# RicoFio/disentangle_mlp

Measured on AMD Instinct MI355X. Metric: celeba64_betavaegan_train_images_per_sec, higher is better.
Workload: dtype fp32-equivalent (fp16x3 split of fp32 operands on the f16 MFMA, fp32 accumulate, every convolution and the Linear layers with >= 2^20 weights (vg_gemm_nt_f16x3); the small Linear layers (vendor GEMMs), BatchNorm, losses, Adam in fp32)

## Files before the change

disentangle_mlp_amd/csrc/common.hpp:

```cpp
#pragma once
#include <hip/hip_runtime.h>
#include <stdint.h>

typedef float f32x16 __attribute__((ext_vector_type(16)));
typedef float f32x4 __attribute__((ext_vector_type(4)));

#define VG_WAVE 64

#ifdef VG_TUNING
#define VG_KNOB(type, name, value) type name = value
#else
#define VG_KNOB(type, name, value) constexpr type name = value
#endif

#define VG_CHECK_LAUNCH()                         \
  do {                                            \
    hipError_t e__ = hipGetLastError();           \
    if (e__ != hipSuccess) return (int)e__;       \
  } while (0)

__device__ __forceinline__ f32x16 mfma32(float a, float b, f32x16 c) {
  return __builtin_amdgcn_mfma_f32_32x32x2f32(a, b, c, 0, 0, 0);
}

__device__ __forceinline__ int acc_row(int r, int lane) {
  return (r & 3) + 8 * (r >> 2) + 4 * (lane >> 5);
}

__device__ __forceinline__ float act_slope(float v, float slope) { return v * (v > 0.f ? 1.f : slope); }

typedef __attribute__((ext_vector_type(8))) __bf16 bf16x8;
typedef __attribute__((ext_vector_type(8))) _Float16 f16x8;

#define VG_PLANES_F16_FLAG 0x100

constexpr int VG_PACK_SPARE = 6;
constexpr size_t vg_pack_trailer_units(int nsteps, int planes, int CoutP) {
  return (size_t)(nsteps + VG_PACK_SPARE) * planes * 2 * CoutP;
}

constexpr int VG_STATS_SLOT_DEPTH = 16;

__device__ __forceinline__ unsigned f16_bound_exp(float amax) {
  const unsigned e = (__float_as_uint(amax) >> 23) & 0xffu;
  return min(max(e, 15u), 254u);
}
__device__ __forceinline__ float f16_scale_of(float amax) { return __uint_as_float((268u - f16_bound_exp(amax)) << 23); }
__device__ __forceinline__ float f16_unscale_of(float amax) { return __uint_as_float((f16_bound_exp(amax) - 14u) << 23); }

template <int NP, bool F16>
__device__ __forceinline__ void split_planes16(float* v, f32x4* out) {
  if constexpr (F16) {
    static_assert(NP == 2, "fp16 planes: hi + lo");
    typedef float f32x2 __attribute__((ext_vector_type(2)));
    typedef _Float16 f16x2 __attribute__((ext_vector_type(2)));
    f16x2 hi[4], lo[4];
#pragma unroll
    for (int j = 0; j < 4; ++j) {
      const f32x2 v2 = {v[2 * j], v[2 * j + 1]};
      const f16x2 h = __builtin_convertvector(v2, f16x2);
      hi[j] = h;
      lo[j] = __builtin_convertvector(v2 - __builtin_convertvector(h, f32x2), f16x2);
    }
    struct P4 { f16x2 q[4]; };
    out[0] = __builtin_bit_cast(f32x4, P4{{hi[0], hi[1], hi[2], hi[3]}});
    out[1] = __builtin_bit_cast(f32x4, P4{{lo[0], lo[1], lo[2], lo[3]}});
  } else {
#pragma unroll
    for (int p = 0; p < NP; ++p) {
      bf16x8 q;
#pragma unroll
      for (int j = 0; j < 8; ++j) {
        const __bf16 h = (__bf16)v[j];
        q[j] = h;
        v[j] -= (float)h;
      }
      out[p] = __builtin_bit_cast(f32x4, q);
    }
  }
}

template <bool F16>
__device__ __forceinline__ f32x16 mfma_split16(bf16x8 a, bf16x8 b, f32x16 c) {
  if constexpr (F16)
    return __builtin_amdgcn_mfma_f32_32x32x16_f16(__builtin_bit_cast(f16x8, a), __builtin_bit_cast(f16x8, b), c, 0, 0, 0);
  else
    return __builtin_amdgcn_mfma_f32_32x32x16_bf16(a, b, c, 0, 0, 0);
}

template <typename T>
__device__ __forceinline__ T wave_sum(T v) {
#pragma unroll
  for (int o = 32; o > 0; o >>= 1) v += __shfl_down(v, o, 64);
  return v;
}

template <typename T>
__device__ __forceinline__ T wave_allsum(T v) {
#pragma unroll
  for (int o = 32; o > 0; o >>= 1) v += __shfl_xor(v, o, 64);
  return v;
}

template <int NT, typename T>
__device__ __forceinline__ T block_sum(T v, T* red) {
  v = wave_sum(v);
  const int lane = threadIdx.x & 63, wid = threadIdx.x >> 6;
  __syncthreads();
  if (lane == 0) red[wid] = v;
  __syncthreads();
  T t = 0;
  if (threadIdx.x == 0) {
#pragma unroll
    for (int i = 0; i < NT / 64; ++i) t += red[i];
  }
  return t;
}

__device__ __forceinline__ unsigned abs_bits(float v) { return __float_as_uint(v) & 0x7fffffffu; }

template <int NT>
__device__ __forceinline__ void block_amax_atomic(unsigned m, unsigned* out) {
  __shared__ unsigned amax_red[NT / 64];
#pragma unroll
  for (int o = 32; o > 0; o >>= 1) m = max(m, (unsigned)__shfl_xor((int)m, o, 64));
  const int lane = threadIdx.x & 63, wid = threadIdx.x >> 6;
  if (lane == 0) amax_red[wid] = m;
  __syncthreads();
  if (threadIdx.x == 0) {
#pragma unroll
    for (int i = 1; i < NT / 64; ++i) m = max(m, amax_red[i]);
    if (m > __hip_atomic_load(out, __ATOMIC_RELAXED, __HIP_MEMORY_SCOPE_AGENT)) atomicMax(out, m);
  }
}

__host__ __device__ constexpr int cdiv(int a, int b) { return (a + b - 1) / b; }

int vg_internal_wgrad_reduce(const float* slabs, float* dw, int n, int splits, hipStream_t st, int accumulate = 0);
size_t vg_internal_ring_workspace_bytes(int mode, int B, int Cin, int H, int W, int Cout, int planes);
size_t vg_internal_ring_stats_floats(int mode, int B, int Cin, int H, int W, int Cout, int planes);
int vg_internal_ring_conv(int mode, const float* x, const void* packed, const float* bias, float* y, int B, int Cin, int H,
                          int W, int Cout, int planes, void* workspace, size_t workspace_bytes, const float* in_scale,
                          const float* in_shift, int in_act, float* stats, size_t stats_floats, const float* in_amax,
                          hipStream_t st);
#ifdef VG_TUNING
void vg_internal_ring_set_variant(int v);
void vg_internal_wx_set_th(int th);
#endif
int vg_internal_convT_s1_thin(const float* x, const float* w, const float* bias, float* y, int B, int Cin, int H,
                              int W, int Cout, hipStream_t st);
```

disentangle_mlp_amd/csrc/conv_ring.hip:

```cpp
#include "common.hpp"
#include "vaegan_hip.h"

namespace {

enum { R_FWD = 0, R_TR = 1 };
constexpr int RNT = 512;
#ifndef VG_RING_SLOTS
#define VG_RING_SLOTS 3
#endif
#ifndef VG_RING_NOPF
#define VG_RING_NOPF 0
#endif
constexpr int ring_slots(bool f16, int slotu, int patchu) {
  if (!f16) return 3;
  int n = VG_RING_SLOTS;
  while (n > 3 && (n * slotu + patchu + 1) * 16 > 160 * 1024) --n;
  return n;
}
static_assert(VG_RING_SLOTS >= 3 && VG_RING_SLOTS <= VG_PACK_SPARE, "ring depth");

constexpr int ring_cols(int mode, int TW, int PW) {
  if (mode == R_FWD) {
    const int need = (PW + 1) / 2;
    if (TW == 8) { int c = need; while ((c & 3) != 2) ++c; return c; }
    return (need + 3) & ~3;
  }
  if (TW == 16) return (PW + 15) & ~15;
  if (TW == 8) { int c = PW; while ((c & 15) != 8) ++c; return c; }
  return (PW + 3) & ~3;
}

template <int MODE_, int NB_, int TH_, int TW_, int WC_, int FC_, int FP_, int NP_, bool F16_ = false>
struct RCfg {
  static constexpr int MODE = MODE_, NB = NB_, TH = TH_, TW = TW_, WC = WC_, WP = 8 / WC_, FC = FC_, FP = FP_, NP = NP_;
  static constexpr bool F16 = F16_;
  static_assert(!F16_ || NP_ == 2, "fp16 planes: hi + lo");
  static constexpr int S = 2;
  static constexpr int TN = 32 * WC * FC, TM = NB * TH * TW;
  static constexpr int NTMAX = (MODE == R_FWD) ? 5 : 3;
  static constexpr int PH = (MODE == R_FWD) ? S * (TH - 1) + 5 : TH + NTMAX - 1;
  static constexpr int PW = (MODE == R_FWD) ? S * (TW - 1) + 5 : TW + NTMAX - 1;
  static constexpr int COLS = ring_cols(MODE, TW, PW);
  static constexpr int ROWU = (MODE == R_FWD) ? 2 * COLS : COLS;
  static constexpr int IMGU = NB * PH * ROWU;
  static constexpr int BUFU = (MODE == R_FWD) ? NP * IMGU : NP * 2 * IMGU;
  static constexpr int PATCHU = 2 * BUFU;
  static constexpr int SLOTU = NP * 2 * TN;
  static constexpr int NSLOT = ring_slots(F16_, SLOTU, PATCHU);
  static constexpr int RINGU = NSLOT * SLOTU;
  static constexpr int LDSU = RINGU + PATCHU + 1;
  static constexpr int DMA_TOTAL = SLOTU / 64;
  static constexpr int NDMA = (DMA_TOTAL + 7) / 8;
  static constexpr int NPIX = NB * PH * PW;
  static constexpr int NQ = ((MODE == R_FWD) ? 1 : 2) * ((NPIX + RNT - 1) / RNT);
  static constexpr int NL = NQ * 8;
  static constexpr int NCLS = (MODE == R_FWD) ? 1 : 4;
  static_assert(TM == 32 * WP * FP, "pixel tile");
  static_assert(FP + 5 <= VG_STATS_SLOT_DEPTH, "statistics slot: an fma chain of FP, 5 butterfly additions");
  static_assert(WC == 1 || WC == 2 || WC == 4 || WC == 8, "wavefront grid");
  static_assert(SLOTU % 64 == 0, "a step's filter slice is whole DMA instructions");
  static_assert(LDSU * 16 <= 160 * 1024, "LDS");
};

struct RArgs {
  const float* x;
  const bf16x8* w;
  const float* bias;
  float* y;
  int B, Cin, XH, XW, Cout, CoutP, YH, YW;
  int ntiles_n, tiles_w, tiles_hw, blocks_per_cls;
  int cps;
  size_t ysplit;
  const float* in_scale;
  const float* in_shift;
  int in_act;
  float* stats;
  const float* in_amax;
  const float* w_unscale;
  int paired;
};

__host__ __device__ constexpr int tr_taps_before(int R, int SS) {
  int n = 0;
  for (int r = 0; r < 2; ++r)
    for (int s = 0; s < 2; ++s) {
      if (r == R && s == SS) return n;
      n += ((5 - r + 1) / 2) * ((5 - s + 1) / 2);
    }
  return n;
}

template <int N>
__device__ __forceinline__ void wait_vmcnt() {
  static_assert(N >= 0 && N < 64, "vmcnt is a 6-bit counter");
  asm volatile("s_waitcnt vmcnt(%0)" ::"n"(N) : "memory");
}

template <class C, int R, int SS, bool AFF, int R2 = -1, int SS2 = -1>
__device__ __forceinline__ void ring_body(const RArgs& A, f32x4* lds, int bid, int split) {
  constexpr int MODE = C::MODE, S = C::S, NB = C::NB, TH = C::TH, TW = C::TW, PH = C::PH, PW = C::PW;
  constexpr int COLS = C::COLS, ROWU = C::ROWU, IMGU = C::IMGU, NQ = C::NQ, FC = C::FC, FP = C::FP, NP = C::NP;
  constexpr int NTMAX = C::NTMAX, BUFU = C::BUFU, SLOTU = C::SLOTU, NDMA = C::NDMA, NL = C::NL, TN = C::TN;
  constexpr int NSLOT = C::NSLOT;
  constexpr bool F16 = C::F16;
  constexpr int NTH = (MODE == R_FWD) ? 5 : (5 - R + 1) / 2;
  constexpr int NTW = (MODE == R_FWD) ? 5 : (5 - SS + 1) / 2;
  constexpr bool TWO = R2 >= 0;
  static_assert(!TWO || MODE == R_TR, "two classes: transposed form");
  constexpr int NTH2 = TWO ? (5 - R2 + 1) / 2 : 0, NTW2 = TWO ? (5 - SS2 + 1) / 2 : 1;
  constexpr int NA = NTH * NTW, NB2 = NTH2 * NTW2;
  constexpr int NSTEP = NA + NB2;
  constexpr int NACC = TWO ? 2 : 1;
  static_assert(!TWO || NA >= NSLOT, "the prologue's DMAs all belong to the first class");
  constexpr int PSTEP = (MODE == R_FWD) ? S : 1;
  constexpr int RING0 = 0, PATCH0 = C::RINGU, DUMMY = C::RINGU + C::PATCHU;

  const int tid = threadIdx.x, lane = tid & 63;
  const int wid = __builtin_amdgcn_readfirstlane(tid >> 6);
  const int kb = lane >> 5, l32 = lane & 31;
  const int wc = wid % C::WC, wp = wid / C::WC;
  int nt, pt;
  {
    const int ntn = A.ntiles_n, npatch = A.blocks_per_cls / ntn, full = (npatch / 8) * 8 * ntn;
    if (bid < full) {
      const int xcd = bid & 7, j = bid >> 3;
      pt = xcd * (npatch / 8) + j / ntn;
      nt = j % ntn;
    } else {
      const int t = bid - full;
      pt = (npatch / 8) * 8 + t / ntn;
      nt = t % ntn;
    }
  }
  const int sp = pt % A.tiles_hw, bg = pt / A.tiles_hw;
  const int th0 = (sp / A.tiles_w) * TH, tw0 = (sp % A.tiles_w) * TW;
  const int b0 = bg * NB, n0 = nt * TN;
  const int Cin = A.Cin, Cout = A.Cout, XH = A.XH, XW = A.XW, HW = XH * XW;
  const int ih0 = (MODE == R_FWD) ? th0 * S - 2 : th0 - (NTMAX - 1 - 2 / S);
  const int iw0 = (MODE == R_FWD) ? tw0 * S - 2 : tw0 - (NTMAX - 1 - 2 / S);
  const float* xb = A.x + (size_t)b0 * Cin * HW;

  struct Unit {
    unsigned ofs;
    int dst;
    bool ok;
  };
  auto unit_of = [&](int q) -> Unit {
    int t0 = tid;
    asm volatile("" : "+v"(t0));
    const int kbs = (MODE == R_FWD) ? 0 : (q & 1);
    const int e = t0 + ((MODE == R_FWD) ? q : (q >> 1)) * RNT;
    const int col = e % PW;
    int t = e / PW;
    const int r = t % PH;
    t /= PH;
    const int nb = t % NB;
    const int ih = ih0 + r, iw = iw0 + col;
    const bool in = e < C::NPIX;
    Unit u;
    u.ok = in && ih >= 0 && ih < XH && iw >= 0 && iw < XW && (b0 + nb) < A.B;
    const int nbc = min(nb, A.B - 1 - b0), ihc = min(max(ih, 0), XH - 1), iwc = min(max(iw, 0), XW - 1);
    u.ofs = 4u * (unsigned)((nbc * Cin + kbs * 8) * HW + ihc * XW + iwc);
    u.dst = in ? kbs * IMGU + (nb * PH + r) * ROWU + ((MODE == R_FWD) ? (col & 1) * COLS + (col >> 1) : col) : -1;
    return u;
  };

  float preg[NQ][8];
  int staged_c0 = 0;
  const float aff_slope = A.in_act == VG_ACT_NONE ? 1.f : (A.in_act == VG_ACT_RELU ? 0.f : 0.2f);
  float x_scale = 1.f, x_unscale = 1.f;
  if constexpr (F16) {
    const float amax = *A.in_amax;
    x_scale = f16_scale_of(amax);
    x_unscale = f16_unscale_of(amax);
  }
  auto stage_load = [&](int c0) {
    c0 = min(c0, Cin - ((MODE == R_FWD) ? 8 : 16));
    staged_c0 = c0;
    unsigned ofs[NQ];
#pragma unroll
    for (int q = 0; q < NQ; ++q) ofs[q] = unit_of(q).ofs;
#pragma unroll
    for (int j = 0; j < 8; ++j) {
      const char* xj = (const char*)(xb + (size_t)(c0 + j) * HW);
#pragma unroll
      for (int q = 0; q < NQ; ++q) preg[q][j] = *(const float*)(xj + ofs[q]);
    }
  };
  auto split_unit = [&](int q, int bufu) {
    const Unit u = unit_of(q);
    f32x4 pl[NP];
    float vv[8];
    const int cb = __builtin_amdgcn_readfirstlane(staged_c0 + ((MODE == R_FWD) ? 0 : (q & 1) * 8));
#pragma unroll
    for (int j = 0; j < 8; ++j) {
      float v = preg[q][j];
      if constexpr (AFF) {
        v = fmaf(v, A.in_scale[cb + j], A.in_shift[cb + j]);
        v = act_slope(v, aff_slope);
      }
      v = u.ok ? v : 0.f;
      vv[j] = F16 ? v * x_scale : v;
    }
    split_planes16<NP, F16>(vv, pl);
    const int d = PATCH0 + bufu + u.dst;
#pragma unroll
    for (int p = 0; p < NP; ++p)
      lds[(u.dst >= 0) ? d + p * ((MODE == R_FWD) ? IMGU : 2 * IMGU) : DUMMY] = pl[p];
  };
  auto stage_store = [&](int bufu) {
#pragma unroll
    for (int q = 0; q < NQ; ++q) split_unit(q, bufu);
  };

  const int CoutP = A.CoutP;
  const size_t wstep = (size_t)2 * NP * CoutP;
  const int nchunks = Cin / 16;
  const bf16x8* wcls = A.w + (size_t)((MODE == R_FWD) ? 0 : tr_taps_before(R, SS)) * nchunks * wstep;
  const bf16x8* dma_ptr2 = A.w + (size_t)(TWO ? tr_taps_before(R2 < 0 ? 0 : R2, SS2 < 0 ? 0 : SS2) : 0) * nchunks * wstep;
  unsigned dma_src[NDMA];
  int dma_dst[NDMA];
#pragma unroll
  for (int j = 0; j < NDMA; ++j) {
    const int i = (wid * NDMA + j) % C::DMA_TOTAL;
    const int u = i * 64 + lane;
    const int row = u / TN, col = u % TN;
    dma_src[j] = 16u * (unsigned)(row * CoutP + n0 + col);
    dma_dst[j] = i * 64;
  }
  const bf16x8* dma_ptr1 = wcls;
  auto dma_next = [&](int slot, bool second = false) {
    const bf16x8*& dma_ptr = second ? dma_ptr2 : dma_ptr1;
#pragma unroll
    for (int j = 0; j < NDMA; ++j) {
      const unsigned m0v = (unsigned)(size_t)(__attribute__((address_space(3))) void*)(lds + RING0 + slot * SLOTU + dma_dst[j]);
      asm volatile("s_mov_b32 m0, %2\n\tglobal_load_lds_dwordx4 %0, %1" ::"v"(dma_src[j]), "s"(dma_ptr), "s"(m0v) : "memory", "m0");
    }
    dma_ptr += wstep;
  };
  int base_a[FC], base_b[FP];
#pragma unroll
  for (int g = 0; g < FC; ++g) base_a[g] = RING0 + kb * TN + (wc * FC + g) * 32 + l32;
#pragma unroll
  for (int f = 0; f < FP; ++f) {
    const int m = (wp * FP + f) * 32 + l32;
    const int nb = m / (TH * TW), r = m % (TH * TW);
    base_b[f] = PATCH0 + (nb * PH + PSTEP * (r / TW)) * ROWU + r % TW + ((MODE == R_TR) ? kb * IMGU : 0);
  }

  f32x16 accs[NACC][FC][FP];
#pragma unroll
  for (int a = 0; a < NACC; ++a)
#pragma unroll
    for (int g = 0; g < FC; ++g)
#pragma unroll
      for (int f = 0; f < FP; ++f)
#pragma unroll
        for (int r = 0; r < 16; ++r) accs[a][g][f][r] = 0.f;

  const int c_begin = split * A.cps, c_end = min(c_begin + A.cps, nchunks);
  const int nsteps = (c_end - c_begin) * NSTEP;

  auto fwd_tap_off = [](int t) constexpr { return (t / 5) * ROWU + ((t % 5) & 1) * COLS + ((t % 5) >> 1); };
  auto step_off = [&](int s, int k) constexpr -> int {
    if constexpr (MODE == R_FWD) {
      const int half = (s < 12) ? 0 : (s == 12 ? k : 1);
      const int tap = (s < 12) ? 2 * s + k : (s == 12 ? 24 : 2 * (s - 13) + k);
      return half * BUFU + fwd_tap_off(tap);
    } else {
      if (TWO && s >= NA) return (NTMAX - 1 - (s - NA) / NTW2) * ROWU + (NTMAX - 1 - (s - NA) % NTW2);
      return (NTMAX - 1 - s / NTW) * ROWU + (NTMAX - 1 - s % NTW);
    }
  };

  bf16x8 av[2][FC][NP], bv[2][FP][NP];
  constexpr int NRD = (FC + FP) * NP;
  auto read_one = [&](int buf, int j, int so, int bo) {
    if (j < FC * NP) {
      const int g = j / NP, p = j % NP;
      av[buf][g][p] = __builtin_bit_cast(bf16x8, lds[base_a[g] + so + p * 2 * TN]);
    } else {
      const int f = (j - FC * NP) / NP, p = (j - FC * NP) % NP;
      bv[buf][f][p] = __builtin_bit_cast(bf16x8, lds[base_b[f] + bo + p * ((MODE == R_FWD) ? IMGU : 2 * IMGU)]);
    }
  };
  auto patch_off = [&](int s, int pbuf) -> int {
    if constexpr (MODE == R_FWD) return kb ? step_off(s, 1) : step_off(s, 0);
    else return pbuf + step_off(s, 0);
  };
  constexpr int NPROD = NP * (NP + 1) / 2, NMF = NPROD * FC * FP;
  auto mfma_one = [&](int buf, int i, int a = 0) {
    auto& acc = accs[a];
    const int pr = i / (FC * FP), g = (i / FP) % FC, f = i % FP;
    int pa = 0, pb = 0, n = 0;
#pragma unroll
    for (int sum = NP - 1; sum >= 0; --sum)
#pragma unroll
      for (int a = sum; a >= 0; --a) {
        if (n == pr) { pa = a; pb = sum - a; }
        ++n;
      }
    acc[g][f] = mfma_split16<F16>(av[buf][g][pa], bv[buf][f][pb], acc[g][f]);
  };
  constexpr int RS = (NMF / NRD) > 0 ? (NMF / NRD) : 1;
  dma_ptr1 += (size_t)c_begin * NA * wstep;
  dma_ptr2 += (size_t)c_begin * NB2 * wstep;
#pragma unroll
  for (int i = 0; i < NSLOT - (VG_RING_NOPF ? 1 : 0); ++i) dma_next(i);
  stage_load(c_begin * 16);
  stage_store(0);
  wait_vmcnt<0>();
  __syncthreads();
  if (!VG_RING_NOPF) {
#pragma unroll
    for (int j = 0; j < NRD; ++j) read_one(0, j, 0, patch_off(0, 0));
  }
  asm volatile("s_waitcnt lgkmcnt(0)" ::: "memory");

#ifdef VG_RING_STAMP
  unsigned long long tk_a = 0, tk_b = 0, tk_c = 0, tk_d = 0, sum_bar = 0, sum_mf = 0, sum_tail = 0, sum_all = 0;
  unsigned long long tm[NMF < 12 ? NMF : 12];
#pragma unroll
  for (int i = 0; i < NMF && i < 12; ++i) tm[i] = 0;
#endif
  int slot = 0;
  for (int ch = c_begin; ch < c_end; ++ch) {
    const int pcur = (MODE == R_TR) ? ((ch - c_begin) & 1) * BUFU : 0;
    const int pnxt = (MODE == R_TR) ? BUFU - pcur : 0;
#pragma unroll
    for (int s = 0; s < NSTEP; ++s) {
      const int cur = s & 1, nxt = cur ^ 1;
      constexpr int LW = (NSTEP >= 6) ? 3 : 2;
      const bool ld = (MODE == R_FWD) ? (s == 0 || s == 13) : (s == 0);
      const bool wr = (MODE == R_FWD) ? (s == 4 || s == 17) : (s == LW);
      const int wbuf = (MODE == R_FWD) ? (s == 4 ? BUFU : 0) : pnxt;
#ifdef VG_RING_STAMP
      asm volatile("s_memtime %0" : "=s"(tk_a));
#endif
      __builtin_amdgcn_s_barrier();
#ifdef VG_RING_STAMP
      asm volatile("s_memtime %0" : "=s"(tk_b));
#endif
      __builtin_amdgcn_sched_barrier(0);
      const int nslot = (slot == NSLOT - 1) ? 0 : slot + 1;
      const int so = nslot * SLOTU;
      const int bo = (s + 1 < NSTEP) ? patch_off(s + 1, pcur) : patch_off(0, pnxt);
      if (VG_RING_NOPF) {
#pragma unroll
        for (int j = 0; j < NRD; ++j) read_one(cur, j, slot * SLOTU, patch_off(s, pcur));
        __builtin_amdgcn_sched_barrier(0);
      }
      auto mem_block = [&]() {
        if constexpr (VG_RING_NOPF != 0)
          dma_next(slot == 0 ? NSLOT - 1 : slot - 1, TWO && (s + NSLOT - 1) % NSTEP >= NA);
        else
          dma_next(slot, TWO && (s + NSLOT) % NSTEP >= NA);
        if (ld) {
          if constexpr (MODE == R_FWD) stage_load(ch * 16 + (s == 0 ? 8 : 16));
          else stage_load((ch + 1) * 16);
        }
      };
#pragma unroll
      for (int i = 0; i < NMF; ++i) {
        mfma_one(cur, i, (TWO && s >= NA) ? 1 : 0);
#ifdef VG_RING_STAMP
        if (i < 12) asm volatile("s_memtime %0" : "=s"(tm[i]));
#endif
        if (i == 0 || i == NMF / 2) {
          if (i == 0) mem_block();
          __builtin_amdgcn_sched_barrier(0);
        }
        if (!VG_RING_NOPF && i % RS == RS - 1 && i / RS < NRD) {
          read_one(nxt, i / RS, so, bo);
          __builtin_amdgcn_sched_barrier(0);
        }
        if (wr && i >= NMF / 2 && (i - NMF / 2) < NQ) {
          split_unit(i - NMF / 2, wbuf);
          __builtin_amdgcn_sched_barrier(0);
        }
      }
#pragma unroll
      for (int j = NMF / RS; j < NRD && !VG_RING_NOPF; ++j) read_one(nxt, j, so, bo);
      if (wr) {
#pragma unroll
        for (int q = NMF - NMF / 2; q < NQ; ++q) split_unit(q, wbuf);
      }
      __builtin_amdgcn_sched_barrier(0);
#ifdef VG_RING_STAMP
      asm volatile("s_memtime %0" : "=s"(tk_c));
#endif
      const bool ldw = (MODE == R_FWD) ? ((s >= 0 && s < NSLOT - 1) || (s >= 13 && s < 13 + NSLOT - 1)) : (s >= 0 && s < NSLOT - 1);
      if (ldw) wait_vmcnt<(NSLOT - 2) * NDMA + NL>(); else wait_vmcnt<(NSLOT - 2) * NDMA>();
      asm volatile("s_waitcnt lgkmcnt(0)" ::: "memory");
#ifdef VG_RING_STAMP
      asm volatile("s_memtime %0\n\ts_waitcnt lgkmcnt(0)" : "=s"(tk_d), "+s"(tk_a), "+s"(tk_b), "+s"(tk_c));
      static_assert(NMF == 12 || NMF == 6 || NMF == 24, "stamp pinning below");
      if constexpr (NMF >= 12)
        asm volatile("" : "+s"(tm[0]), "+s"(tm[1]), "+s"(tm[2]), "+s"(tm[3]), "+s"(tm[4]), "+s"(tm[5]), "+s"(tm[6]), "+s"(tm[7]),
                     "+s"(tm[8]), "+s"(tm[9]), "+s"(tm[10]), "+s"(tm[11]));
      else
        asm volatile("" : "+s"(tm[0]), "+s"(tm[1]), "+s"(tm[2]), "+s"(tm[3]), "+s"(tm[4]), "+s"(tm[5]));
      sum_bar += tk_b - tk_a;
      sum_mf += tk_c - tk_b;
      sum_tail += tk_d - tk_c;
      sum_all += 1;
#endif
      __builtin_amdgcn_sched_barrier(0);
      slot = nslot;
    }
    if constexpr (NSTEP & 1) {
#pragma unroll
      for (int p = 0; p < NP; ++p) {
#pragma unroll
        for (int g = 0; g < FC; ++g) av[0][g][p] = av[1][g][p];
#pragma unroll
        for (int f = 0; f < FP; ++f) bv[0][f][p] = bv[1][f][p];
      }
    }
  }
  wait_vmcnt<0>();
  if constexpr (F16) {
    const float w_unscale = *A.w_unscale;
#pragma unroll
    for (int a = 0; a < NACC; ++a)
#pragma unroll
      for (int g = 0; g < FC; ++g)
#pragma unroll
        for (int f = 0; f < FP; ++f)
#pragma unroll
          for (int r = 0; r < 16; ++r) accs[a][g][f][r] = accs[a][g][f][r] * x_unscale * w_unscale;
  }

  const int YH = A.YH, YW = A.YW;
#ifdef VG_RING_STAMP
  if (A.stats && lane == 0 && bid < 64) {
    unsigned long long* o = (unsigned long long*)A.stats + (size_t)(bid * 8 + wid) * 4;
    o[0] = sum_bar; o[1] = sum_mf; o[2] = sum_tail; o[3] = sum_all;
    unsigned long long* o2 = (unsigned long long*)A.stats + 64 * 8 * 4 + (size_t)(bid * 8 + wid) * 16;
    o2[0] = tk_a; o2[1] = tk_b; o2[2] = tk_c; o2[3] = tk_d;
#pragma unroll
    for (int i = 0; i < NMF && i < 12; ++i) o2[4 + i] = tm[i];
  }
  const bool emit_stats = false;
#else
  const bool emit_stats = A.stats != nullptr;
#endif
  auto emit = [&](auto& acc, int Rc, int SSc) {
  if (emit_stats) {
    bool pokf[FP];
#pragma unroll
    for (int f = 0; f < FP; ++f) {
      const int m = (wp * FP + f) * 32 + l32;
      const int nb = m / (TH * TW), r = m % (TH * TW);
      const int th = th0 + r / TW, tw = tw0 + r % TW;
      const int oh = (MODE == R_FWD) ? th : S * th + Rc, ow = (MODE == R_FWD) ? tw : S * tw + SSc;
      pokf[f] = (b0 + nb) < A.B && oh < YH && ow < YW;
    }
    const int cls = (MODE == R_FWD) ? 0 : 2 * Rc + SSc;
    const int slot = (cls * (A.blocks_per_cls / A.ntiles_n) + pt) * C::WP + wp;
    float* sb = A.stats + (size_t)slot * Cout * 2;
#pragma unroll
    for (int g = 0; g < FC; ++g)
#pragma unroll
      for (int r16 = 0; r16 < 16; ++r16) {
        const int co = n0 + (wc * FC + g) * 32 + acc_row(r16, lane);
        const float bvs = A.bias ? A.bias[min(co, Cout - 1)] : 0.f;
        float s1 = 0.f, s2 = 0.f;
#pragma unroll
        for (int f = 0; f < FP; ++f) {
          const float v = pokf[f] ? acc[g][f][r16] + bvs : 0.f;
          s1 += v;
          s2 = fmaf(v, v, s2);
        }
#pragma unroll
        for (int o = 16; o > 0; o >>= 1) {
          s1 += __shfl_xor(s1, o, 64);
          s2 += __shfl_xor(s2, o, 64);
        }
        if (l32 == 0 && co < Cout) {
          sb[2 * co] = s1;
          sb[2 * co + 1] = s2;
        }
      }
  }
#pragma unroll
  for (int f = 0; f < FP; ++f) {
    const int m = (wp * FP + f) * 32 + l32;
    const int nb = m / (TH * TW), r = m % (TH * TW);
    const int th = th0 + r / TW, tw = tw0 + r % TW, b = b0 + nb;
    const int oh = (MODE == R_FWD) ? th : S * th + Rc;
    const int ow = (MODE == R_FWD) ? tw : S * tw + SSc;
    const bool pok = b < A.B && oh < YH && ow < YW;
    float* yb = A.y + (size_t)split * A.ysplit + ((size_t)b * Cout * YH + oh) * YW + ow;
#pragma unroll
    for (int g = 0; g < FC; ++g) {
      float bvv[16];
#pragma unroll
      for (int r16 = 0; r16 < 16; ++r16) {
        const int co = min(n0 + (wc * FC + g) * 32 + acc_row(r16, lane), Cout - 1);
        bvv[r16] = (A.bias && split == 0) ? A.bias[co] : 0.f;
      }
#pragma unroll
      for (int r16 = 0; r16 < 16; ++r16) {
        const int co = n0 + (wc * FC + g) * 32 + acc_row(r16, lane);
        if (pok && co < Cout) yb[(size_t)co * YH * YW] = acc[g][f][r16] + bvv[r16];
      }
    }
  }
  };
  emit(accs[0], R, SS);
  if constexpr (TWO) emit(accs[1], R2, SS2);
}

template <class C, bool AFF>
__global__ __launch_bounds__(RNT, 2) void conv5x5_ring_kernel(RArgs A) {
  __shared__ f32x4 lds[C::LDSU];
  int bid = blockIdx.x;
  if constexpr (C::NCLS == 1) {
    const int split = bid / A.blocks_per_cls;
    ring_body<C, 0, 0, AFF>(A, lds, bid - split * A.blocks_per_cls, split);
  } else {
    const int per = A.blocks_per_cls;
    if (A.paired) {
      const int nsplit = gridDim.x / (2 * per);
      const int xcd = bid & 7, j = bid >> 3;
      const int pair = j & 1;
      bid = (j >> 1) * 8 + xcd;
      const int split = bid / per;
      bid -= split * per;
      if constexpr (C::F16) {
        if (pair == 0) ring_body<C, 0, 0, AFF, 1, 1>(A, lds, bid, split);
        else ring_body<C, 0, 1, AFF, 1, 0>(A, lds, bid, split);
      }
      return;
    }
    const int nsplit = gridDim.x / (4 * per);
    const int cls = bid / (per * nsplit);
    bid -= cls * per * nsplit;
    const int split = bid / per;
    bid -= split * per;
    switch (cls) {
      case 0: ring_body<C, 0, 0, AFF>(A, lds, bid, split); break;
      case 1: ring_body<C, 0, 1, AFF>(A, lds, bid, split); break;
      case 2: ring_body<C, 1, 0, AFF>(A, lds, bid, split); break;
      default: ring_body<C, 1, 1, AFF>(A, lds, bid, split); break;
    }
  }
}

struct RFuse {
  const float* in_scale;
  const float* in_shift;
  int in_act;
  float* stats;
  const float* in_amax;
};

template <class C>
int launch_ring(const float* x, const bf16x8* w, const float* bias, float* y, int B, int Cin, int XH, int XW, int Cout,
                int ksplit, float* slabs, RFuse fu, hipStream_t st) {
  RArgs A;
  A.x = x; A.w = w; A.bias = bias; A.y = y;
  A.in_scale = fu.in_scale; A.in_shift = fu.in_shift; A.in_act = fu.in_act;
  A.stats = (ksplit == 1) ? fu.stats : nullptr;
  A.in_amax = fu.in_amax;
  A.B = B; A.Cin = Cin; A.XH = XH; A.XW = XW; A.Cout = Cout; A.CoutP = (Cout + 127) & ~127;
  A.w_unscale = (const float*)(w + vg_pack_trailer_units(Cin / 16 * 25, C::NP, A.CoutP));
  int tsh, tsw;
  if (C::MODE == R_FWD) {
    A.YH = (XH - 1) / 2 + 1; A.YW = (XW - 1) / 2 + 1;
    tsh = A.YH; tsw = A.YW;
  } else {
    A.YH = XH * 2; A.YW = XW * 2;
    tsh = XH; tsw = XW;
  }
  A.tiles_w = cdiv(tsw, C::TW);
  A.tiles_hw = cdiv(tsh, C::TH) * A.tiles_w;
  A.ntiles_n = cdiv(Cout, C::TN);
  const long per_cls = (long)A.ntiles_n * A.tiles_hw * cdiv(B, C::NB);
  A.paired = (C::NCLS == 4 && C::F16 && per_cls * ksplit * 2 >= 256 && per_cls % 8 == 0) ? 1 : 0;
  const long grid = per_cls * (A.paired ? 2 : C::NCLS) * ksplit;
  if (grid <= 0 || grid > 0x7fffffffL) return VG_ERR_BAD_ARG;
  A.blocks_per_cls = (int)per_cls;
  A.cps = cdiv(Cin / 16, ksplit);
  A.ysplit = (size_t)B * Cout * A.YH * A.YW;
  if (ksplit > 1) A.y = slabs;
  if (A.in_scale) hipLaunchKernelGGL((conv5x5_ring_kernel<C, true>), dim3((unsigned)grid), dim3(RNT), 0, st, A);
  else hipLaunchKernelGGL((conv5x5_ring_kernel<C, false>), dim3((unsigned)grid), dim3(RNT), 0, st, A);
// ... 117 lines not shown
```

Measured before the change: 9369.

## Use 16x16x32 fp16 MFMA with paired-step double slots in ring conv

```diff
diff --git a/disentangle_mlp_amd/csrc/common.hpp b/disentangle_mlp_amd/csrc/common.hpp
--- a/disentangle_mlp_amd/csrc/common.hpp
+++ b/disentangle_mlp_amd/csrc/common.hpp
@@ -88,6 +88,14 @@
     return __builtin_amdgcn_mfma_f32_32x32x16_bf16(a, b, c, 0, 0, 0);
 }
 
+template <bool F16>
+__device__ __forceinline__ f32x4 mfma_split16_k32(bf16x8 a, bf16x8 b, f32x4 c) {
+  if constexpr (F16)
+    return __builtin_amdgcn_mfma_f32_16x16x32_f16(__builtin_bit_cast(f16x8, a), __builtin_bit_cast(f16x8, b), c, 0, 0, 0);
+  else
+    return __builtin_amdgcn_mfma_f32_16x16x32_bf16(a, b, c, 0, 0, 0);
+}
+
 template <typename T>
 __device__ __forceinline__ T wave_sum(T v) {
 #pragma unroll
diff --git a/disentangle_mlp_amd/csrc/conv_ring.hip b/disentangle_mlp_amd/csrc/conv_ring.hip
--- a/disentangle_mlp_amd/csrc/conv_ring.hip
+++ b/disentangle_mlp_amd/csrc/conv_ring.hip
@@ -1,23 +1,13 @@
 #include "common.hpp"
 #include "vaegan_hip.h"
 
+#include <type_traits>
+
 namespace {
 
 enum { R_FWD = 0, R_TR = 1 };
 constexpr int RNT = 512;
-#ifndef VG_RING_SLOTS
-#define VG_RING_SLOTS 3
-#endif
-#ifndef VG_RING_NOPF
-#define VG_RING_NOPF 0
-#endif
-constexpr int ring_slots(bool f16, int slotu, int patchu) {
-  if (!f16) return 3;
-  int n = VG_RING_SLOTS;
-  while (n > 3 && (n * slotu + patchu + 1) * 16 > 160 * 1024) --n;
-  return n;
-}
-static_assert(VG_RING_SLOTS >= 3 && VG_RING_SLOTS <= VG_PACK_SPARE, "ring depth");
+constexpr int ring_slots(bool f16) { return f16 ? 6 : 3; }
 
 constexpr int ring_cols(int mode, int TW, int PW) {
   if (mode == R_FWD) {
@@ -29,6 +19,7 @@
   if (TW == 8) { int c = PW; while ((c & 15) != 8) ++c; return c; }
   return (PW + 3) & ~3;
 }
+__host__ __device__ constexpr int k32_pixel(int r) { return r < 4 ? 2 * r : (r >= 12 ? 2 * (r - 8) : 2 * (r - 4) + 1); }
 
 template <int MODE_, int NB_, int TH_, int TW_, int WC_, int FC_, int FP_, int NP_, bool F16_ = false>
 struct RCfg {
@@ -46,9 +37,9 @@
   static constexpr int BUFU = (MODE == R_FWD) ? NP * IMGU : NP * 2 * IMGU;
   static constexpr int PATCHU = 2 * BUFU;
   static constexpr int SLOTU = NP * 2 * TN;
-  static constexpr int NSLOT = ring_slots(F16_, SLOTU, PATCHU);
+  static constexpr int NSLOT = ring_slots(F16_);
   static constexpr int RINGU = NSLOT * SLOTU;
-  static constexpr int LDSU = RINGU + PATCHU + 1;
+  static constexpr int LDSU = RINGU + PATCHU + (F16_ ? 2 : 1);
   static constexpr int DMA_TOTAL = SLOTU / 64;
   static constexpr int NDMA = (DMA_TOTAL + 7) / 8;
   static constexpr int NPIX = NB * PH * PW;
@@ -56,9 +47,13 @@
   static constexpr int NL = NQ * 8;
   static constexpr int NCLS = (MODE == R_FWD) ? 1 : 4;
   static_assert(TM == 32 * WP * FP, "pixel tile");
-  static_assert(FP + 5 <= VG_STATS_SLOT_DEPTH, "statistics slot: an fma chain of FP, 5 butterfly additions");
+  static_assert((F16_ ? 2 * FP + 4 : FP + 5) <= VG_STATS_SLOT_DEPTH, "statistics slot depth");
   static_assert(WC == 1 || WC == 2 || WC == 4 || WC == 8, "wavefront grid");
   static_assert(SLOTU % 64 == 0, "a step's filter slice is whole DMA instructions");
+  static_assert(NSLOT <= VG_PACK_SPARE, "ring depth against the pack's spare steps");
+  static_assert(!F16_ || (TN % 16 == 0 && SLOTU % 16 == 0 && COLS % 2 == 0 && ROWU % 2 == 0 && IMGU % 2 == 0 && BUFU % 2 == 0),
+                "K = 32 body: LDS bank rules of ring_cols");
+  static_assert(!F16_ || TW == 16 || (TW == 8 && (((MODE == R_FWD) ? S : 1) * ROWU) % 16 == 8), "K = 32 body: a fragment's 16 pixels");
   static_assert(LDSU * 16 <= 160 * 1024, "LDS");
 };
 
@@ -106,18 +101,21 @@
   constexpr int NTH = (MODE == R_FWD) ? 5 : (5 - R + 1) / 2;
   constexpr int NTW = (MODE == R_FWD) ? 5 : (5 - SS + 1) / 2;
   constexpr bool TWO = R2 >= 0;
-  static_assert(!TWO || MODE == R_TR, "two classes: transposed form");
+  static_assert(!TWO || (MODE == R_TR && F16), "two classes: transposed form, fp16 planes (with three planes two accumulator sets spill)");
   constexpr int NTH2 = TWO ? (5 - R2 + 1) / 2 : 0, NTW2 = TWO ? (5 - SS2 + 1) / 2 : 1;
   constexpr int NA = NTH * NTW, NB2 = NTH2 * NTW2;
   constexpr int NSTEP = NA + NB2;
   constexpr int NACC = TWO ? 2 : 1;
-  static_assert(!TWO || NA >= NSLOT, "the prologue's DMAs all belong to the first class");
   constexpr int PSTEP = (MODE == R_FWD) ? S : 1;
-  constexpr int RING0 = 0, PATCH0 = C::RINGU, DUMMY = C::RINGU + C::PATCHU;
+  constexpr int PLANEU = (MODE == R_FWD) ? IMGU : 2 * IMGU;
+  constexpr int RING0 = 0, PATCH0 = C::RINGU, DUMMY = C::RINGU + C::PATCHU, ZEROU = DUMMY + 1;
+  constexpr int FR = F16 ? 16 : 32, AG = (32 / FR) * FC, AF = (32 / FR) * FP, NR = FR * FR / 64;
+  using Acc = std::conditional_t<F16, f32x4, f32x16>;
 
   const int tid = threadIdx.x, lane = tid & 63;
   const int wid = __builtin_amdgcn_readfirstlane(tid >> 6);
   const int kb = lane >> 5, l32 = lane & 31;
+  const int kq = lane >> 4, l16 = lane & 15;
   const int wc = wid % C::WC, wp = wid / C::WC;
   int nt, pt;
   {
@@ -205,8 +203,7 @@
     split_planes16<NP, F16>(vv, pl);
     const int d = PATCH0 + bufu + u.dst;
 #pragma unroll
-    for (int p = 0; p < NP; ++p)
-      lds[(u.dst >= 0) ? d + p * ((MODE == R_FWD) ? IMGU : 2 * IMGU) : DUMMY] = pl[p];
+    for (int p = 0; p < NP; ++p) lds[(u.dst >= 0) ? d + p * PLANEU : DUMMY] = pl[p];
   };
   auto stage_store = [&](int bufu) {
 #pragma unroll
@@ -238,28 +235,28 @@
     }
     dma_ptr += wstep;
   };
-  int base_a[FC], base_b[FP];
-#pragma unroll
-  for (int g = 0; g < FC; ++g) base_a[g] = RING0 + kb * TN + (wc * FC + g) * 32 + l32;
-#pragma unroll
-  for (int f = 0; f < FP; ++f) {
-    const int m = (wp * FP + f) * 32 + l32;
+  const int frow = F16 ? l16 : l32, fpix = F16 ? k32_pixel(l16) : l32;
+  int base_a[AG], base_b[AF];
+#pragma unroll
+  for (int g = 0; g < AG; ++g) base_a[g] = RING0 + (F16 ? 0 : kb * TN) + wc * FC * 32 + g * FR + frow;
+#pragma unroll
+  for (int f = 0; f < AF; ++f) {
+    const int m = wp * FP * 32 + f * FR + fpix;
     const int nb = m / (TH * TW), r = m % (TH * TW);
-    base_b[f] = PATCH0 + (nb * PH + PSTEP * (r / TW)) * ROWU + r % TW + ((MODE == R_TR) ? kb * IMGU : 0);
-  }
-
-  f32x16 accs[NACC][FC][FP];
+    base_b[f] = PATCH0 + (nb * PH + PSTEP * (r / TW)) * ROWU + r % TW + ((MODE == R_TR) ? (F16 ? (kq & 1) : kb) * IMGU : 0);
+  }
+
+  Acc accs[NACC][AG][AF];
 #pragma unroll
   for (int a = 0; a < NACC; ++a)
 #pragma unroll
-    for (int g = 0; g < FC; ++g)
-#pragma unroll
-      for (int f = 0; f < FP; ++f)
-#pragma unroll
-        for (int r = 0; r < 16; ++r) accs[a][g][f][r] = 0.f;
+    for (int g = 0; g < AG; ++g)
+#pragma unroll
+      for (int f = 0; f < AF; ++f)
+#pragma unroll
+        for (int r = 0; r < NR; ++r) accs[a][g][f][r] = 0.f;
 
   const int c_begin = split * A.cps, c_end = min(c_begin + A.cps, nchunks);
-  const int nsteps = (c_end - c_begin) * NSTEP;
 
   auto fwd_tap_off = [](int t) constexpr { return (t / 5) * ROWU + ((t % 5) & 1) * COLS + ((t % 5) >> 1); };
   auto step_off = [&](int s, int k) constexpr -> int {
@@ -272,149 +269,208 @@
       return (NTMAX - 1 - s / NTW) * ROWU + (NTMAX - 1 - s % NTW);
     }
   };
-
-  bf16x8 av[2][FC][NP], bv[2][FP][NP];
-  constexpr int NRD = (FC + FP) * NP;
-  auto read_one = [&](int buf, int j, int so, int bo) {
-    if (j < FC * NP) {
-      const int g = j / NP, p = j % NP;
-      av[buf][g][p] = __builtin_bit_cast(bf16x8, lds[base_a[g] + so + p * 2 * TN]);
-    } else {
-      const int f = (j - FC * NP) / NP, p = (j - FC * NP) % NP;
-      bv[buf][f][p] = __builtin_bit_cast(bf16x8, lds[base_b[f] + bo + p * ((MODE == R_FWD) ? IMGU : 2 * IMGU)]);
-    }
-  };
-  auto patch_off = [&](int s, int pbuf) -> int {
-    if constexpr (MODE == R_FWD) return kb ? step_off(s, 1) : step_off(s, 0);
-    else return pbuf + step_off(s, 0);
-  };
-  constexpr int NPROD = NP * (NP + 1) / 2, NMF = NPROD * FC * FP;
-  auto mfma_one = [&](int buf, int i, int a = 0) {
-    auto& acc = accs[a];
-    const int pr = i / (FC * FP), g = (i / FP) % FC, f = i % FP;
-    int pa = 0, pb = 0, n = 0;
-#pragma unroll
+  constexpr int NPROD = NP * (NP + 1) / 2;
+  auto prod_planes = [](int pr, int& pa, int& pb) constexpr {
+    int n = 0;
     for (int sum = NP - 1; sum >= 0; --sum)
-#pragma unroll
       for (int a = sum; a >= 0; --a) {
         if (n == pr) { pa = a; pb = sum - a; }
         ++n;
       }
-    acc[g][f] = mfma_split16<F16>(av[buf][g][pa], bv[buf][f][pb], acc[g][f]);
-  };
-  constexpr int RS = (NMF / NRD) > 0 ? (NMF / NRD) : 1;
+  };
+
   dma_ptr1 += (size_t)c_begin * NA * wstep;
   dma_ptr2 += (size_t)c_begin * NB2 * wstep;
-#pragma unroll
-  for (int i = 0; i < NSLOT - (VG_RING_NOPF ? 1 : 0); ++i) dma_next(i);
-  stage_load(c_begin * 16);
-  stage_store(0);
-  wait_vmcnt<0>();
-  __syncthreads();
-  if (!VG_RING_NOPF) {
+
+  if constexpr (F16) {
+    constexpr int DA = (NA + 1) / 2, DB = (NB2 + 1) / 2, NDB = DA + DB;
+    static_assert(NSLOT == 6 && NP == 2, "three double slots, hi + lo");
+    static_assert(NDB >= 2 && (!TWO || DA >= 2), "the prologue's two DMAs belong to the first class of the first chunk");
+    auto second_of = [](int d) constexpr { return TWO && d >= DA; };
+    auto step0_of = [](int d) constexpr { return (TWO && d >= DA) ? NA + 2 * (d - DA) : 2 * d; };
+    auto half_of = [](int d) constexpr { return (TWO && d >= DA) ? 2 * (d - DA) + 1 >= NB2 : 2 * d + 1 >= NA; };
+    auto dma_body = [&](int ds, int e) {
+      dma_next(2 * ds, second_of(e));
+      dma_next(2 * ds + 1, second_of(e));
+      if (half_of(e)) (second_of(e) ? dma_ptr2 : dma_ptr1) -= wstep;
+    };
+    const int aoff0 = (kq >> 1) * SLOTU + (kq & 1) * TN;
+    const int aoff1 = (kq & 1) * SLOTU + (((kq + 1) >> 1) & 1) * TN;
+    bf16x8 av[AG][NP], bv[AF][NP];
+    constexpr int NMF = NPROD * AG * AF;
+
+    if (tid == 0) lds[ZEROU] = f32x4{0.f, 0.f, 0.f, 0.f};
+    dma_body(0, 0);
+    dma_body(1, 1);
+    stage_load(c_begin * 16);
+    stage_store(0);
+    wait_vmcnt<0>();
+    __syncthreads();
+
+    int slot = 0;
+    for (int ch = c_begin; ch < c_end; ++ch) {
+      const int pcur = (MODE == R_TR) ? ((ch - c_begin) & 1) * BUFU : 0;
+      const int pnxt = (MODE == R_TR) ? BUFU - pcur : 0;
+#pragma unroll
+      for (int d = 0; d < NDB; ++d) {
+        constexpr int WRD = (NDB >= 3) ? 2 : 1;
+        const bool ld = (MODE == R_FWD) ? (d == 0 || d == 7) : (d == 0);
+        const bool wr = (MODE == R_FWD) ? (d == 2 || d == 9) : (d == WRD);
+        const int wbuf = (MODE == R_FWD) ? (d == 2 ? BUFU : 0) : pnxt;
+        __builtin_amdgcn_s_barrier();
+        __builtin_amdgcn_sched_barrier(0);
+        const bool half = half_of(d);
+        const int s0 = step0_of(d);
+        const int o0 = step_off(s0, 0), o1 = step_off(s0, 1);
+        const int o2 = half ? o0 : step_off(s0 + 1, 0), o3 = half ? o1 : step_off(s0 + 1, 1);
+        const bool perm = MODE == R_FWD && !half && ((o0 ^ o3) & 1) + ((o1 ^ o2) & 1) < ((o0 ^ o1) & 1) + ((o2 ^ o3) & 1);
+        int bo;
+        if constexpr (MODE == R_FWD) {
+          const int q1 = perm ? o3 : o1, q2 = perm ? o1 : o2, q3 = perm ? o2 : o3;
+          bo = kq == 0 ? o0 : (kq == 1 ? q1 : (kq == 2 ? q2 : q3));
+        } else {
+          bo = pcur + ((kq >> 1) ? o2 : o0);
+        }
+        const int sa = slot * (2 * SLOTU) + (perm ? aoff1 : aoff0);
+#pragma unroll
+        for (int h = 0; h < 2; ++h) {
+          const int pa = h ? 0 : 1, pb = h ? 1 : 0;
+#pragma unroll
+          for (int g = 0; g < AG; ++g) av[g][pa] = __builtin_bit_cast(bf16x8, lds[base_a[g] + sa + pa * 2 * TN]);
+#pragma unroll
+          for (int f = 0; f < AF; ++f) {
+            int bi = base_b[f] + bo + pb * PLANEU;
+            if (half) bi = (kq >= 2) ? ZEROU : bi;
+            bv[f][pb] = __builtin_bit_cast(bf16x8, lds[bi]);
+          }
+        }
+        __builtin_amdgcn_sched_barrier(0);
+        const int e = (d + 2) % NDB;
+#pragma unroll
+        for (int i = 0; i < NMF; ++i) {
+          const int pr = i / (AG * AF), g = (i / AF) % AG, f = i % AF;
+          int pa = 0, pb = 0;
+          prod_planes(pr, pa, pb);
+          Acc& acc = accs[second_of(d) ? 1 : 0][g][f];
+          acc = mfma_split16_k32<true>(av[g][pa], bv[f][pb], acc);
+          if (i == 0) {
+            dma_body(slot == 0 ? 2 : slot - 1, e);
+            if (ld) {
+              if constexpr (MODE == R_FWD) stage_load(ch * 16 + (d == 0 ? 8 : 16));
+              else stage_load((ch + 1) * 16);
+            }
+            __builtin_amdgcn_sched_barrier(0);
+          }
+          if (wr && i >= NMF / 2 && (i - NMF / 2) < NQ) {
+            __builtin_amdgcn_sched_barrier(0);
+            split_unit(i - NMF / 2, wbuf);
+            __builtin_amdgcn_sched_barrier(0);
+          }
+        }
+        static_assert(NQ <= NMF - NMF / 2, "a staging event's units fit between the later MFMAs");
+        __builtin_amdgcn_sched_barrier(0);
+        const bool ldw = (MODE == R_FWD) ? (d == 0 || d == 1 || d == 7 || d == 8) : (d < WRD);
+        if (ldw) wait_vmcnt<2 * NDMA + NL>(); else wait_vmcnt<2 * NDMA>();
+        asm volatile("s_waitcnt lgkmcnt(0)" ::: "memory");
+        __builtin_amdgcn_sched_barrier(0);
+        slot = (slot == 2) ? 0 : slot + 1;
+      }
+    }
+  } else {
+    static_assert(!TWO, "two classes per workgroup: K = 32 body only");
+    bf16x8 av[2][FC][NP], bv[2][FP][NP];
+    constexpr int NRD = (FC + FP) * NP;
+    auto read_one = [&](int buf, int j, int so, int bo) {
+      if (j < FC * NP) {
+        const int g = j / NP, p = j % NP;
+        av[buf][g][p] = __builtin_bit_cast(bf16x8, lds[base_a[g] + so + p * 2 * TN]);
+      } else {
+        const int f = (j - FC * NP) / NP, p = (j - FC * NP) % NP;
+        bv[buf][f][p] = __builtin_bit_cast(bf16x8, lds[base_b[f] + bo + p * PLANEU]);
+      }
+    };
+    auto patch_off = [&](int s, int pbuf) -> int {
+      if constexpr (MODE == R_FWD) return kb ? step_off(s, 1) : step_off(s, 0);
+      else return pbuf + step_off(s, 0);
+    };
+    constexpr int NMF = NPROD * FC * FP;
+    auto mfma_one = [&](int buf, int i) {
+      const int pr = i / (FC * FP), g = (i / FP) % FC, f = i % FP;
+      int pa = 0, pb = 0;
+      prod_planes(pr, pa, pb);
+      accs[0][g][f] = mfma_split16<false>(av[buf][g][pa], bv[buf][f][pb], accs[0][g][f]);
+    };
+    constexpr int RS = (NMF / NRD) > 0 ? (NMF / NRD) : 1;
+#pragma unroll
+    for (int i = 0; i < NSLOT; ++i) dma_next(i);
+    stage_load(c_begin * 16);
+    stage_store(0);
+    wait_vmcnt<0>();
+    __syncthreads();
 #pragma unroll
     for (int j = 0; j < NRD; ++j) read_one(0, j, 0, patch_off(0, 0));
-  }
-  asm volatile("s_waitcnt lgkmcnt(0)" ::: "memory");
-
-#ifdef VG_RING_STAMP
-  unsigned long long tk_a = 0, tk_b = 0, tk_c = 0, tk_d = 0, sum_bar = 0, sum_mf = 0, sum_tail = 0, sum_all = 0;
-  unsigned long long tm[NMF < 12 ? NMF : 12];
-#pragma unroll
-  for (int i = 0; i < NMF && i < 12; ++i) tm[i] = 0;
-#endif
-  int slot = 0;
-  for (int ch = c_begin; ch < c_end; ++ch) {
-    const int pcur = (MODE == R_TR) ? ((ch - c_begin) & 1) * BUFU : 0;
-    const int pnxt = (MODE == R_TR) ? BUFU - pcur : 0;
-#pragma unroll
-    for (int s = 0; s < NSTEP; ++s) {
-      const int cur = s & 1, nxt = cur ^ 1;
-      constexpr int LW = (NSTEP >= 6) ? 3 : 2;
-      const bool ld = (MODE == R_FWD) ? (s == 0 || s == 13) : (s == 0);
-      const bool wr = (MODE == R_FWD) ? (s == 4 || s == 17) : (s == LW);
-      const int wbuf = (MODE == R_FWD) ? (s == 4 ? BUFU : 0) : pnxt;
-#ifdef VG_RING_STAMP
-      asm volatile("s_memtime %0" : "=s"(tk_a));
-#endif
-      __builtin_amdgcn_s_barrier();
-#ifdef VG_RING_STAMP
-      asm volatile("s_memtime %0" : "=s"(tk_b));
-#endif
-      __builtin_amdgcn_sched_barrier(0);
-      const int nslot = (slot == NSLOT - 1) ? 0 : slot + 1;
-      const int so = nslot * SLOTU;
-      const int bo = (s + 1 < NSTEP) ? patch_off(s + 1, pcur) : patch_off(0, pnxt);
-      if (VG_RING_NOPF) {
-#pragma unroll
-        for (int j = 0; j < NRD; ++j) read_one(cur, j, slot * SLOTU, patch_off(s, pcur));
+    asm volatile("s_waitcnt lgkmcnt(0)" ::: "memory");
+
+    int slot = 0;
+    for (int ch = c_begin; ch < c_end; ++ch) {
+      const int pcur = (MODE == R_TR) ? ((ch - c_begin) & 1) * BUFU : 0;
+      const int pnxt = (MODE == R_TR) ? BUFU - pcur : 0;
+#pragma unroll
+      for (int s = 0; s < NSTEP; ++s) {
+        const int cur = s & 1, nxt = cur ^ 1;
+        constexpr int LW = (NSTEP >= 6) ? 3 : 2;
+        const bool ld = (MODE == R_FWD) ? (s == 0 || s == 13) : (s == 0);
+        const bool wr = (MODE == R_FWD) ? (s == 4 || s == 17) : (s == LW);
+        const int wbuf = (MODE == R_FWD) ? (s == 4 ? BUFU : 0) : pnxt;
+        __builtin_amdgcn_s_barrier();
         __builtin_amdgcn_sched_barrier(0);
-      }
-      auto mem_block = [&]() {
-        if constexpr (VG_RING_NOPF != 0)
-          dma_next(slot == 0 ? NSLOT - 1 : slot - 1, TWO && (s + NSLOT - 1) % NSTEP >= NA);
-        else
-          dma_next(slot, TWO && (s + NSLOT) % NSTEP >= NA);
-        if (ld) {
-          if constexpr (MODE == R_FWD) stage_load(ch * 16 + (s == 0 ? 8 : 16));
-          else stage_load((ch + 1) * 16);
-        }
-      };
-#pragma unroll
-      for (int i = 0; i < NMF; ++i) {
-        mfma_one(cur, i, (TWO && s >= NA) ? 1 : 0);
-#ifdef VG_RING_STAMP
-        if (i < 12) asm volatile("s_memtime %0" : "=s"(tm[i]));
-#endif
-        if (i == 0 || i == NMF / 2) {
-          if (i == 0) mem_block();
-          __builtin_amdgcn_sched_barrier(0);
-        }
-        if (!VG_RING_NOPF && i % RS == RS - 1 && i / RS < NRD) {
-          read_one(nxt, i / RS, so, bo);
-          __builtin_amdgcn_sched_barrier(0);
-        }
-        if (wr && i >= NMF / 2 && (i - NMF / 2) < NQ) {
-          split_unit(i - NMF / 2, wbuf);
-          __builtin_amdgcn_sched_barrier(0);
-        }
-      }
-#pragma unroll
-      for (int j = NMF / RS; j < NRD && !VG_RING_NOPF; ++j) read_one(nxt, j, so, bo);
-      if (wr) {
-#pragma unroll
-        for (int q = NMF - NMF / 2; q < NQ; ++q) split_unit(q, wbuf);
-      }
-      __builtin_amdgcn_sched_barrier(0);
-#ifdef VG_RING_STAMP
-      asm volatile("s_memtime %0" : "=s"(tk_c));
-#endif
-      const bool ldw = (MODE == R_FWD) ? ((s >= 0 && s < NSLOT - 1) || (s >= 13 && s < 13 + NSLOT - 1)) : (s >= 0 && s < NSLOT - 1);
-      if (ldw) wait_vmcnt<(NSLOT - 2) * NDMA + NL>(); else wait_vmcnt<(NSLOT - 2) * NDMA>();
-      asm volatile("s_waitcnt lgkmcnt(0)" ::: "memory");
-#ifdef VG_RING_STAMP
-      asm volatile("s_memtime %0\n\ts_waitcnt lgkmcnt(0)" : "=s"(tk_d), "+s"(tk_a), "+s"(tk_b), "+s"(tk_c));
-      static_assert(NMF == 12 || NMF == 6 || NMF == 24, "stamp pinning below");
-      if constexpr (NMF >= 12)
-        asm volatile("" : "+s"(tm[0]), "+s"(tm[1]), "+s"(tm[2]), "+s"(tm[3]), "+s"(tm[4]), "+s"(tm[5]), "+s"(tm[6]), "+s"(tm[7]),
-                     "+s"(tm[8]), "+s"(tm[9]), "+s"(tm[10]), "+s"(tm[11]));
-      else
-        asm volatile("" : "+s"(tm[0]), "+s"(tm[1]), "+s"(tm[2]), "+s"(tm[3]), "+s"(tm[4]), "+s"(tm[5]));
-      sum_bar += tk_b - tk_a;
-      sum_mf += tk_c - tk_b;
-      sum_tail += tk_d - tk_c;
-      sum_all += 1;
-#endif
-      __builtin_amdgcn_sched_barrier(0);
-      slot = nslot;
-    }
-    if constexpr (NSTEP & 1) {
-#pragma unroll
-      for (int p = 0; p < NP; ++p) {
-#pragma unroll
-        for (int g = 0; g < FC; ++g) av[0][g][p] = av[1][g][p];
-#pragma unroll
-        for (int f = 0; f < FP; ++f) bv[0][f][p] = bv[1][f][p];
+        const int nslot = (slot == NSLOT - 1) ? 0 : slot + 1;
+        const int so = nslot * SLOTU;
+        const int bo = (s + 1 < NSTEP) ? patch_off(s + 1, pcur) : patch_off(0, pnxt);
+        auto mem_block = [&]() {
+          dma_next(slot);
+          if (ld) {
+            if constexpr (MODE == R_FWD) stage_load(ch * 16 + (s == 0 ? 8 : 16));
+            else stage_load((ch + 1) * 16);
+          }
+        };
+#pragma unroll
+        for (int i = 0; i < NMF; ++i) {
+          mfma_one(cur, i);
+          if (i == 0 || i == NMF / 2) {
+            if (i == 0) mem_block();
+            __builtin_amdgcn_sched_barrier(0);
+          }
+          if (i % RS == RS - 1 && i / RS < NRD) {
+            read_one(nxt, i / RS, so, bo);
+            __builtin_amdgcn_sched_barrier(0);
+          }
+          if (wr && i >= NMF / 2 && (i - NMF / 2) < NQ) {
+            split_unit(i - NMF / 2, wbuf);
+            __builtin_amdgcn_sched_barrier(0);
+          }
+        }
+#pragma unroll
+        for (int j = NMF / RS; j < NRD; ++j) read_one(nxt, j, so, bo);
+        if (wr) {
+#pragma unroll
+          for (int q = NMF - NMF / 2; q < NQ; ++q) split_unit(q, wbuf);
+        }
+        __builtin_amdgcn_sched_barrier(0);
+        const bool ldw = (MODE == R_FWD) ? ((s >= 0 && s < NSLOT - 1) || (s >= 13 && s < 13 + NSLOT - 1)) : (s >= 0 && s < NSLOT - 1);
+        if (ldw) wait_vmcnt<(NSLOT - 2) * NDMA + NL>(); else wait_vmcnt<(NSLOT - 2) * NDMA>();
+        asm volatile("s_waitcnt lgkmcnt(0)" ::: "memory");
+        __builtin_amdgcn_sched_barrier(0);
+        slot = nslot;
+      }
+      if constexpr (NSTEP & 1) {
+#pragma unroll
+        for (int p = 0; p < NP; ++p) {
+#pragma unroll
+          for (int g = 0; g < FC; ++g) av[0][g][p] = av[1][g][p];
+#pragma unroll
+          for (int f = 0; f < FP; ++f) bv[0][f][p] = bv[1][f][p];
+        }
       }
     }
   }
@@ -424,33 +480,22 @@
 #pragma unroll
     for (int a = 0; a < NACC; ++a)
 #pragma unroll
-      for (int g = 0; g < FC; ++g)
-#pragma unroll
-        for (int f = 0; f < FP; ++f)
-#pragma unroll
-          for (int r = 0; r < 16; ++r) accs[a][g][f][r] = accs[a][g][f][r] * x_unscale * w_unscale;
-  }
-
+      for (int g = 0; g < AG; ++g)
+#pragma unroll
+        for (int f = 0; f < AF; ++f)
+#pragma unroll
+          for (int r = 0; r < NR; ++r) accs[a][g][f][r] = accs[a][g][f][r] * x_unscale * w_unscale;
+  }
+
+  auto row_of = [&](int g, int r) { return n0 + wc * FC * 32 + g * FR + (F16 ? 4 * kq + r : acc_row(r, lane)); };
   const int YH = A.YH, YW = A.YW;
-#ifdef VG_RING_STAMP
-  if (A.stats && lane == 0 && bid < 64) {
-    unsigned long long* o = (unsigned long long*)A.stats + (size_t)(bid * 8 + wid) * 4;
-    o[0] = sum_bar; o[1] = sum_mf; o[2] = sum_tail; o[3] = sum_all;
-    unsigned long long* o2 = (unsigned long long*)A.stats + 64 * 8 * 4 + (size_t)(bid * 8 + wid) * 16;
-    o2[0] = tk_a; o2[1] = tk_b; o2[2] = tk_c; o2[3] = tk_d;
-#pragma unroll
-    for (int i = 0; i < NMF && i < 12; ++i) o2[4 + i] = tm[i];
-  }
-  const bool emit_stats = false;
-#else
   const bool emit_stats = A.stats != nullptr;
-#endif
   auto emit = [&](auto& acc, int Rc, int SSc) {
   if (emit_stats) {
-    bool pokf[FP];
-#pragma unroll
-    for (int f = 0; f < FP; ++f) {
-      const int m = (wp * FP + f) * 32 + l32;
+    bool pokf[AF];
+#pragma unroll
+    for (int f = 0; f < AF; ++f) {
+      const int m = wp * FP * 32 + f * FR + fpix;
       const int nb = m / (TH * TW), r = m % (TH * TW);
       const int th = th0 + r / TW, tw = tw0 + r % TW;
       const int oh = (MODE == R_FWD) ? th : S * th + Rc, ow = (MODE == R_FWD) ? tw : S * tw + SSc;
@@ -460,32 +505,32 @@
     const int slot = (cls * (A.blocks_per_cls / A.ntiles_n) + pt) * C::WP + wp;
     float* sb = A.stats + (size_t)slot * Cout * 2;
 #pragma unroll
-    for (int g = 0; g < FC; ++g)
-#pragma unroll
-      for (int r16 = 0; r16 < 16; ++r16) {
-        const int co = n0 + (wc * FC + g) * 32 + acc_row(r16, lane);
+    for (int g = 0; g < AG; ++g)
+#pragma unroll
+      for (int r = 0; r < NR; ++r) {
+        const int co = row_of(g, r);
         const float bvs = A.bias ? A.bias[min(co, Cout - 1)] : 0.f;
         float s1 = 0.f, s2 = 0.f;
 #pragma unroll
-        for (int f = 0; f < FP; ++f) {
-          const float v = pokf[f] ? acc[g][f][r16] + bvs : 0.f;
+        for (int f = 0; f < AF; ++f) {
+          const float v = pokf[f] ? acc[g][f][r] + bvs : 0.f;
           s1 += v;
           s2 = fmaf(v, v, s2);
         }
 #pragma unroll
-        for (int o = 16; o > 0; o >>= 1) {
+        for (int o = FR / 2; o > 0; o >>= 1) {
           s1 += __shfl_xor(s1, o, 64);
           s2 += __shfl_xor(s2, o, 64);
         }
-        if (l32 == 0 && co < Cout) {
+        if (frow == 0 && co < Cout) {
           sb[2 * co] = s1;
           sb[2 * co + 1] = s2;
         }
       }
   }
 #pragma unroll
-  for (int f = 0; f < FP; ++f) {
-    const int m = (wp * FP + f) * 32 + l32;
+  for (int f = 0; f < AF; ++f) {
+    const int m = wp * FP * 32 + f * FR + fpix;
     const int nb = m / (TH * TW), r = m % (TH * TW);
     const int th = th0 + r / TW, tw = tw0 + r % TW, b = b0 + nb;
     const int oh = (MODE == R_FWD) ? th : S * th + Rc;
@@ -493,17 +538,15 @@
     const bool pok = b < A.B && oh < YH && ow < YW;
     float* yb = A.y + (size_t)split * A.ysplit + ((size_t)b * Cout * YH + oh) * YW + ow;
 #pragma unroll
-    for (int g = 0; g < FC; ++g) {
-      float bvv[16];
-#pragma unroll
-      for (int r16 = 0; r16 < 16; ++r16) {
-        const int co = min(n0 + (wc * FC + g) * 32 + acc_row(r16, lane), Cout - 1);
-        bvv[r16] = (A.bias && split == 0) ? A.bias[co] : 0.f;
-      }
-#pragma unroll
-      for (int r16 = 0; r16 < 16; ++r16) {
-        const int co = n0 + (wc * FC + g) * 32 + acc_row(r16, lane);
-        if (pok && co < Cout) yb[(size_t)co * YH * YW] = acc[g][f][r16] + bvv[r16];
+    for (int g = 0; g < AG; ++g) {
+      float bvv[NR];
+#pragma unroll
+      for (int r = 0; r < NR; ++r)
+        bvv[r] = (A.bias && split == 0) ? A.bias[min(row_of(g, r), Cout - 1)] : 0.f;
+#pragma unroll
+      for (int r = 0; r < NR; ++r) {
+        const int co = row_of(g, r);
+        if (pok && co < Cout) yb[(size_t)co * YH * YW] = acc[g][f][r] + bvv[r];
       }
     }
   }
```

Measured after the change: 9294 (median of 2 runs). About the same (-0.8%).
